# anshmehtamm/ripplemq

Hardware: AMD Instinct MI355X
Metric: committed msgs/sec (node) + HBM GB/s, 100B msgs, 4096 partitions RF=3 (higher is better)
Workload: dtype u8

## Files before the change

### ripplemq_amd/csrc/device_common.hpp

```cpp
#pragma once
#include <hip/hip_runtime.h>
#include <stdint.h>

namespace rmq {

typedef uint32_t u32;
typedef uint64_t u64;
typedef __attribute__((address_space(1))) u64 gu64;
typedef __attribute__((address_space(1))) u32 gu32;

__device__ __forceinline__ void store_sc1(u64* p, u64 v) {
  __hip_atomic_store((gu64*)p, v, __ATOMIC_RELAXED, __HIP_MEMORY_SCOPE_AGENT);
}
__device__ __forceinline__ u64 load_sc1(const u64* p) {
  return __hip_atomic_load((gu64*)p, __ATOMIC_RELAXED, __HIP_MEMORY_SCOPE_AGENT);
}

constexpr u32 kCrcPoly = 0x82F63B78u;
constexpr u32 kRecAlign = 16;

struct CrcConsts {
  u32 table[8][256];
  u32 zshift[2][4][256];
  u32 zshift1k[4][256];
  u32 inv_pad[16];
  u32 sh16[64];
  u32 inv_pad16[16];
  u32 nib[16][32];
};

__host__ __device__ __forceinline__ constexpr u32 record_bytes(u32 len) {
  return 16u + ((len + kRecAlign - 1u) & ~(kRecAlign - 1u));
}

typedef u32 u32x4 __attribute__((ext_vector_type(4)));
typedef u32 u32x2 __attribute__((ext_vector_type(2)));

#ifndef RMQ_RING_NT
#define RMQ_RING_NT 1
#endif
#ifndef RMQ_PAYLOAD_NT
#define RMQ_PAYLOAD_NT 1
#endif
__device__ __forceinline__ uint4 load_payload16(const void* src) {
#if RMQ_PAYLOAD_NT
  const u32x4 x = __builtin_nontemporal_load(reinterpret_cast<const u32x4*>(src));
  return make_uint4(x[0], x[1], x[2], x[3]);
#else
  return *reinterpret_cast<const uint4*>(src);
#endif
}

typedef __attribute__((address_space(1))) const u32x4 gu32x4c;
__device__ __forceinline__ uint4 load_payload16g(u64 addr) {
#if RMQ_PAYLOAD_NT
  const u32x4 x = __builtin_nontemporal_load((gu32x4c*)addr);
#else
  const u32x4 x = *(gu32x4c*)addr;
#endif
  return make_uint4(x[0], x[1], x[2], x[3]);
}

__device__ __forceinline__ void store_log16(uint8_t* dst, uint4 v) {
#if RMQ_RING_NT
  const u32x4 x = {v.x, v.y, v.z, v.w};
  __builtin_nontemporal_store(x, reinterpret_cast<u32x4*>(dst));
#else
  *reinterpret_cast<uint4*>(dst) = v;
#endif
}

__device__ __forceinline__ u32 lane_id() { return __builtin_amdgcn_mbcnt_hi(~0u, __builtin_amdgcn_mbcnt_lo(~0u, 0u)); }


__device__ __forceinline__ u32 gf2_mulmod(u32 a, u32 b) {
  u32 p = 0;
#pragma unroll
  for (int k = 31; k >= 0; --k) {
    p ^= b & (0u - ((a >> k) & 1u));
    b = (b >> 1) ^ (kCrcPoly & (0u - (b & 1u)));
  }
  return p;
}

__device__ __forceinline__ u32 gf2_mulmod_half(u32 a16, u32 b) {
  u32 p = 0;
#pragma unroll
  for (int k = 15; k >= 0; --k) {
    p ^= b & (0u - ((a16 >> k) & 1u));
    b = (b >> 1) ^ (kCrcPoly & (0u - (b & 1u)));
  }
  return p;
}

__device__ __forceinline__ u32 crc_step8(const u32 (*t)[256], u32 c, u32 lo, u32 hi) {
  lo ^= c;
  return t[7][lo & 0xFF] ^ t[6][(lo >> 8) & 0xFF] ^ t[5][(lo >> 16) & 0xFF] ^ t[4][lo >> 24] ^
         t[3][hi & 0xFF] ^ t[2][(hi >> 8) & 0xFF] ^ t[1][(hi >> 16) & 0xFF] ^ t[0][hi >> 24];
}

__device__ __forceinline__ u32 crc_zshift(const u32 (*z)[256], u32 c) {
  return z[0][c & 0xFF] ^ z[1][(c >> 8) & 0xFF] ^ z[2][(c >> 16) & 0xFF] ^ z[3][c >> 24];
}

template <u32 kThreads>
__device__ __forceinline__ void crc_nib_lds(const CrcConsts* crc, u32* scratch) {
  static_assert(sizeof(CrcConsts::nib) == 128 * 16 && kThreads >= 128, "one 16-byte block per thread");
  if (threadIdx.x < 128u)
    reinterpret_cast<uint4*>(scratch)[threadIdx.x] = reinterpret_cast<const uint4*>(&crc->nib[0][0])[threadIdx.x];
  __syncthreads();
}
constexpr u32 kNibBlocks = 128u, kPadBlocks = 4u;
template <u32 kThreads>
__device__ __forceinline__ uint4 crc_nib_load(const CrcConsts* crc) {
  static_assert(sizeof(CrcConsts::nib) == kNibBlocks * 16 && kThreads >= kNibBlocks + 2u * kPadBlocks, "one block per thread");
  static_assert(sizeof(CrcConsts::inv_pad) == kPadBlocks * 16 && sizeof(CrcConsts::inv_pad16) == kPadBlocks * 16, "pad tables");
  const u32 t = threadIdx.x;
  uint4 v = make_uint4(0, 0, 0, 0);
  if (t < kNibBlocks + 2u * kPadBlocks) {
    const uint4* src = t < kNibBlocks ? reinterpret_cast<const uint4*>(&crc->nib[0][0]) + t
                       : t < kNibBlocks + kPadBlocks
                           ? reinterpret_cast<const uint4*>(&crc->inv_pad[0]) + (t - kNibBlocks)
                           : reinterpret_cast<const uint4*>(&crc->inv_pad16[0]) + (t - kNibBlocks - kPadBlocks);
    v = *src;
  }
  return v;
}
__device__ __forceinline__ void crc_nib_put(u32* scratch, u32* pads, uint4 v) {
  const u32 t = threadIdx.x;
  if (t < kNibBlocks)
    reinterpret_cast<uint4*>(scratch)[t] = v;
  else if (t < kNibBlocks + 2u * kPadBlocks)
    reinterpret_cast<uint4*>(pads)[t - kNibBlocks] = v;
}
template <u32 kThreads>
__device__ __forceinline__ void crc_expand_lds(u32* tabs, const u32* scratch) {
  for (u32 b = threadIdx.x; b < 256u; b += kThreads) {
#pragma unroll
    for (u32 q = 0; q < 16u; ++q) tabs[256u * q + b] = scratch[32u * q + (b & 15u)] ^ scratch[32u * q + 16u + (b >> 4)];
  }
}
template <u32 kThreads>
__device__ __forceinline__ void crc_tables_lds(const CrcConsts* crc, u32* tabs, u32* scratch) {
  crc_nib_lds<kThreads>(crc, scratch);
  crc_expand_lds<kThreads>(tabs, scratch);
}

__device__ __forceinline__ u32 crc_piece16(const u32 (*t)[256], uint4 v) {
  return crc_step8(t, crc_step8(t, 0u, v.x, v.y), v.z, v.w);
}

__device__ __forceinline__ u32 pair_swap(u32 v) {
  return (u32)__builtin_amdgcn_update_dpp(0, (int)v, 0xB1, 0xF, 0xF, true);
}


template <int kCtrl, int kRowMask>
__device__ __forceinline__ u32 dpp_mov(u32 v) {
  return (u32)__builtin_amdgcn_update_dpp(0, (int)v, kCtrl, kRowMask, 0xf, true);
}
template <int kCtrl, int kRowMask>
__device__ __forceinline__ u64 dpp_mov(u64 v) {
  return ((u64)dpp_mov<kCtrl, kRowMask>((u32)(v >> 32)) << 32) | dpp_mov<kCtrl, kRowMask>((u32)v);
}

__device__ __forceinline__ u64 bcast_u64(u64 v, u32 l) {
  return ((u64)(u32)__builtin_amdgcn_readlane((int)(v >> 32), (int)l) << 32) |
         (u32)__builtin_amdgcn_readlane((int)(u32)v, (int)l);
}

template <typename T>
__device__ __forceinline__ T wave_incl_scan(T v) {
// ... 84 lines not shown
```

### ripplemq_amd/csrc/engine.cpp

```cpp
#include <chrono>
#include <climits>

#include "engine_internal.hpp"

using namespace rmq;

namespace rmq {

uint32_t host_mulmod(uint32_t a, uint32_t b) {
  uint32_t p = 0;
  for (int k = 31; k >= 0; --k) {
    if ((a >> k) & 1u) p ^= b;
    b = (b >> 1) ^ (kCrcPoly & (0u - (b & 1u)));
  }
  return p;
}

uint32_t host_inverse(uint32_t a) {
  uint32_t col[32];
  for (int k = 0; k < 32; ++k) col[k] = host_mulmod(1u << k, a);
  uint32_t rows[32];
  uint32_t rhs = 0;
  for (int bb = 0; bb < 32; ++bb) {
    rows[bb] = 0;
// ... 19 lines not shown
    ++r;
  }
  uint32_t y = 0;
  for (int q = 0; q < r; ++q)
    if ((rhs >> q) & 1u) y |= 1u << piv[q];
  return y;
}

void build_crc_consts(CrcConsts* c) {
  for (uint32_t b = 0; b < 256; ++b) {
    uint32_t x = b;
    for (int k = 0; k < 8; ++k) x = (x >> 1) ^ (kCrcPoly & (0u - (x & 1u)));
    c->table[0][b] = x;
  }
  for (uint32_t t = 1; t < 8; ++t)
    for (uint32_t b = 0; b < 256; ++b)
      c->table[t][b] = (c->table[t - 1][b] >> 8) ^ c->table[0][c->table[t - 1][b] & 0xFF];
  uint32_t x2n[40];
  x2n[0] = 0x40000000u;
  for (int k = 1; k < 40; ++k) x2n[k] = host_mulmod(x2n[k - 1], x2n[k - 1]);
  for (uint32_t k = 0; k < 2; ++k)
    for (uint32_t i = 0; i < 4; ++i)
      for (uint32_t b = 0; b < 256; ++b) c->zshift[k][i][b] = host_mulmod(b << (8 * i), x2n[7 + k]);
  for (uint32_t i = 0; i < 4; ++i)
    for (uint32_t b = 0; b < 256; ++b) c->zshift1k[i][b] = host_mulmod(b << (8 * i), x2n[13]);
  uint32_t x128e = 0x80000000u;
  for (uint32_t e = 0; e < 64; ++e) {
    c->sh16[e] = x128e;
    x128e = host_mulmod(x128e, x2n[7]);
  }
  uint32_t x8n = 0x80000000u;
  for (uint32_t n = 0; n < 16; ++n) {
    c->inv_pad[n] = n ? host_inverse(x8n) : 0x80000000u;
    c->inv_pad16[n] = host_mulmod(c->inv_pad[n], x2n[4]);
    x8n = host_mulmod(x8n, x2n[3]);
  }
  for (uint32_t q = 0; q < 16; ++q) {
    const uint32_t* t = q < 8 ? c->table[q] : c->zshift[(q - 8) / 4][(q - 8) % 4];
    for (uint32_t n = 0; n < 16; ++n) {
      c->nib[q][n] = t[n];
      c->nib[q][16 + n] = t[n << 4];
    }
  }
}

bool is_pow2(uint64_t v) { return v && !(v & (v - 1)); }

uint32_t ilog2(uint64_t v) {
  uint32_t r = 0;
  while ((1ull << r) < v) ++r;
  return r;
}

int check_err(rmq_engine* e) {
  const hipError_t q = hipStreamQuery(e->main_s);
  return q == hipSuccess || q == hipErrorNotReady ? RMQ_OK : hip_fail(q);
}

template <typename T>
static int spin_then_block(T what, hipError_t (*query)(T), hipError_t (*block)(T)) {
  const auto t0 = std::chrono::steady_clock::now();
  for (;;) {
    const hipError_t q = query(what);
    if (q == hipSuccess) return RMQ_OK;
    if (q != hipErrorNotReady) return hip_fail(q);
    if (std::chrono::steady_clock::now() - t0 > std::chrono::milliseconds(20)) break;
  }
// ... 518 lines not shown
```

### ripplemq_amd/csrc/pipeline.hip

```cpp
#include <hip/hip_ext.h>

#include "device_common.hpp"
#include "kernels.hpp"
#include "partition_ops.hpp"


#ifndef RMQ_PIPE_NS
#define RMQ_PIPE_NS rmq
#endif
namespace RMQ_PIPE_NS {
using namespace rmq;

constexpr u32 kPT = kPipeThreads;
constexpr u32 kPW = kPT / 64;
constexpr u32 kTR = kTileRecs;
constexpr u32 kTI = kTR / kPT;
constexpr u32 kWR = kTR / kPW;
constexpr u32 kIB = kTileIdxBits;
constexpr u32 kFlagShift = 29;
constexpr u32 kRankMask = (1u << kFlagShift) - 1u;
constexpr u32 kFlNoPart = 1u, kFlInvalid = 4u, kFlJunk = 7u;
constexpr u64 kOne40 = 1ull << 40;
constexpr u64 kCnt23 = (1ull << 23) - 1ull;
constexpr u64 kExclNoSpace = 1ull << 63;
constexpr u32 kRejInvalid = 2u;

#define PIPE_STAMP_ROW(row, k)                                                                \
  do {                                                                                        \
    if (A.stamps) {                                                                           \
      const u64 t_ = __builtin_amdgcn_s_memrealtime();                                        \
      if ((threadIdx.x & 63) == 0)                                                            \
        A.stamps[((u64)(row) * kPW + (threadIdx.x >> 6)) * 8 + (k)] = t_;                    \
    }                                                                                         \
  } while (0)
#define PIPE_STAMP(k) PIPE_STAMP_ROW(blockIdx.x, k)

struct Stage1Smem {
  u32 items[2][kTR];
  u32 cnt[kPW][256];
  u32 dbase[256];
  u32 info[kTR];
  u64 wsum[kPW][2];
  u64 wtail[kPW];
  u32 whead[kPW];
  u32 scan[kPW];
};

struct Stage3Smem {
  u32 t8[8][256];
  u32 z[2][4][256];
  uint4 img[kPW][kTaskRecs][8];
  uint4 info[kPW][kTaskRecs];
  u32 pad[2][16];
  union {
    u32 zk[4][256];
    struct {
      u64 xdst[kPW][kTaskRecs][kMaxRemote];
      u32 xn[kPW][kTaskRecs];
    };
  };
};

constexpr size_t kSmemBytes = sizeof(Stage1Smem) > sizeof(Stage3Smem) ? sizeof(Stage1Smem) : sizeof(Stage3Smem);
static_assert(kSmemBytes >= kMaxTiles * sizeof(u64), "stage 2's tile bases fit the dynamic LDS");
static_assert(kPT != 256 || 4 * kSmemBytes <= 160 * 1024, "four 256-thread workgroups per CU fit the 160 KB of LDS");

__device__ __forceinline__ u64 wave_incl_scan_u64(u64 v) { return wave_incl_scan<u64>(v); }

__device__ __forceinline__ u32 record_rs16(u32 L) {
  return (L >> 4) + ((L & 15u) ? 1u : 0u) + 1u;
}

__device__ __forceinline__ u32 batch_of_tile(const PipeGroup& G, u32 t) {
  u32 j = 0;
#pragma unroll
  for (u32 k = 1; k < kMaxGroup; ++k) j += (k < G.nb && t >= G.tile0[k]) ? 1u : 0u;
  return j;
}
__device__ __forceinline__ u32 batch_of_task(const PipeGroup& G, u32 task) {
  u32 j = 0;
#pragma unroll
  for (u32 k = 1; k < kMaxGroup; ++k) j += (k < G.nb && task >= G.task0[k]) ? 1u : 0u;
  return j;
}
__device__ __forceinline__ u32 batch_end_tile(const PipeGroup& G, u32 t) {
  u32 e = G.tiles;
#pragma unroll
  for (int k = (int)kMaxGroup - 1; k >= 1; --k)
    if ((u32)k < G.nb && t < G.tile0[k]) e = G.tile0[k];
  return e;
}

constexpr u32 kBigPieces = 64;
constexpr u32 kBU = 4;

__device__ __forceinline__ u64 readlane64(u64 v, u32 l) {
  return ((u64)(u32)__builtin_amdgcn_readlane((int)(v >> 32), (int)l) << 32) |
         (u32)__builtin_amdgcn_readlane((int)(u32)v, (int)l);
// ... 1343 lines not shown
}

__device__ __forceinline__ void big_close(const PipeArgs& A, const BigRec& R, u32 acc) {
  const u32 lane = threadIdx.x & 63, RF = A.st.RF;
  if (((lane + 64u - R.ph) & 63u) < R.m) {
    const u32 e = (R.m - 1u - lane + R.ph) & 63u;
    if (e) acc = gf2_mulmod(acc, A.crc->sh16[e]);
  }
  acc = wave_xor_all(acc);
  if (lane == 0) {
    const u32 pad = 16u * R.m - R.L;
    const u32 crc = ~(pad ? gf2_mulmod(A.crc->inv_pad[pad], acc) : acc);
    const uint4 h = make_uint4((u32)R.off, (u32)(R.off >> 32), R.L, crc);
    uint8_t* ring = reinterpret_cast<uint8_t*>(R.ring);
    if (R.dead == 0u)
      for (u32 r = 0; r < RF; ++r)
        if ((R.lm >> r) & 1u) store_log16(ring + (R.pos & R.segm) + r * A.st.rstride, h);
#pragma unroll
    for (u32 q = 0; q < kMaxRemote; ++q)
      if (q < R.nx) store_log16(reinterpret_cast<uint8_t*>(R.x[q]), h);
  }
}

template <bool XR>
__device__ __forceinline__ void stage3_big_waves(const PipeArgs& A, Stage3Smem& S, u32 wg) {
  const PipeGroup& G = A.g3;
  const PipeScratch& x = A.s3;
  const DevState& st = A.st;
  const u32 nbig = __builtin_amdgcn_readfirstlane(*reinterpret_cast<volatile const u32*>(x.nbig));
  if (!nbig) return;
  {
    const uint4* src = reinterpret_cast<const uint4*>(&A.crc->table[0][0]);
    uint4* dst = reinterpret_cast<uint4*>(&S.t8[0][0]);
    for (u32 k = threadIdx.x; k < (sizeof(S.t8) + sizeof(S.z)) / 16u; k += kPT) dst[k] = src[k];
    if (!XR) {
      const uint4* zs = reinterpret_cast<const uint4*>(&A.crc->zshift1k[0][0]);
      uint4* zd = reinterpret_cast<uint4*>(&S.zk[0][0]);
      for (u32 k = threadIdx.x; k < sizeof(S.zk) / 16u; k += kPT) zd[k] = zs[k];
    }
  }
  __syncthreads();
  const u32 nw = A.wgb * kPW, lane = threadIdx.x & 63u;
  const u32 e0 = __builtin_amdgcn_readfirstlane(wg * kPW + (threadIdx.x >> 6));
  for (u32 base = e0; base < nbig; base += 64u * nw) {
    const u32 e = base + lane * nw;
    bool ok = e < nbig;
    u64 src = 0, pos = 0, off = 0, ringb = 0, segm = 0;
    u32 L = 0, dead = 0, lm = 0, nx = 0;
    u64 xdst[kMaxRemote] = {};
    if (ok) {
      const u32 gi = x.bigl[e];
      const u32 t = gi / kTR, jb = batch_of_tile(G, t);
      const PipeBatch& b = G.b[jb];
      const u32 i = (t - G.tile0[jb]) * kTR + gi % kTR;
      const uint2 cr = x.crank[gi];
      ok = !(u32)A.s3.binfo[jb * 4] && (cr.x >> kFlagShift) == 0u;
      const u32 p = b.pidx[i];
      L = b.len[i];
      src = reinterpret_cast<u64>(b.payload) + (b.poff ? b.poff[i] : x.tile_base[t] + x.pre[gi]);
      const u64 ex = ok ? x.excl[(u64)p * A.gt + t] : 0ull;
      ok = ok && st.is_leader[p] && !(ex & kExclNoSpace);
      if (ok) {
        const u64 tot = x.totals[p], leo = A.cur.leo[p], used = A.cur.used[p];
        const u32 rk = (u32)((ex >> 40) & kCnt23) + (cr.x & kRankMask);
        const u32 rel16 = (u32)(ex & kLow40) + cr.y;
        off = leo + rk;
        pos = used + 16ull * rel16;
// ... 69 lines not shown

template <bool XR>
__device__ __forceinline__ void stage3_finish(const PipeArgs& A, const Stage3Smem& S, const TaskPos& T, const TaskRec& R,
                              const TaskState& Z, bool cand, uint4& stat_out) {
  const PipeBatch& b = A.g3.b[T.jb];
  const DevState& st = A.st;
  const u32 lane = threadIdx.x & 63, j = lane & 1u;
  const u32 RF = st.RF;
  const u32 i = task_rec(T);
  const bool in = i < b.n;
  const u32 p = R.p, L = R.L;
  const u32 fl = R.cr.x >> kFlagShift;
  const u32 rej = R.rej;
  const bool ns = (Z.lm & kNoSpace) != 0u;
  const bool lead = (Z.lm & kLead) != 0u;
  const u32 lm8 = Z.lm & 0xFFu;
  const bool ok = cand && lead && !ns;
  const u32 m = (L + 15u) >> 4;
  const bool big = ok && m > kBigPieces;
  const bool okp = ok && !big;
  const RingRef rg = ring_ref(Z.rdesc, st.interval_log2, st.icap_mul);
  const u64 segmask = rg.seg - 1ull;
  const u64 rstride = st.rstride;
  const u64 off = Z.off, pos = Z.pos;
  const u32 dead = Z.dead;
  uint8_t* const ring = st.logs + rg.base;
  const u32 lmw = (A.debug & 1u) ? 0u : lm8;
  const u32 sa = (u32)(R.src & 15u);
  u32 acc = 0;
  const u32 nr = okp ? (m + kPR - 1u) / kPR : 0u;
  const bool img = __all(!okp || m <= 7u);
  const u32 w = threadIdx.x >> 6, r32 = lane >> 1;
  Stage3Smem& W = const_cast<Stage3Smem&>(S);
  constexpr bool xr = XR;
  if (xr) {
    if (j == 0) {
      u32 nx = 0;
      if (ok) {
        const u64 rel = 16ull * Z.rel16;
        const u64 rk = Z.rk;
        for (u32 r = 0; r < RF; ++r) {
          if ((lm8 >> r) & 1u) continue;
          const u32 e = A.outidx[(u64)p * RF + r];
          if (e == ~0u) continue;
          const XEntry x = A.xe3[e];
          if (x.data_abs == kNoRound) continue;
          W.xdst[w][r32][nx++] = reinterpret_cast<u64>(A.outbox3 + x.data_abs + rel);
          *reinterpret_cast<u64*>(A.outbox3 + x.tab_abs + 8ull * rk) =
              (u64)x.k | ((u64)(x.data_start16 + (u32)(rel >> 4)) << 32);
        }
      }
      W.xn[w][r32] = nx;
    }
    __builtin_amdgcn_wave_barrier();
  }
  uint4 blk[kBL];
#pragma unroll
  for (u32 q = 0; q < kBL; ++q) blk[q] = Z.blk[q];
  if (Z.nblk) {
    uint4* sg = &W.img[w][0][0];
    static_assert(sizeof(S.img[0]) >= 64u * kSpanPer * 16u, "a wave's image area holds the staged span");
#pragma unroll
    for (u32 u = 0; u < kSpanPer; ++u)
      if (lane + 64u * u < Z.nblk) sg[lane + 64u * u] = Z.blk[u];
    __builtin_amdgcn_wave_barrier();
    const u32 b0 = (u32)(((R.src & ~15ull) - Z.sbase) >> 4) + j;
#pragma unroll
    for (u32 q = 0; q < kBL; ++q) {
      const u32 k = b0 + 2u * q;
      blk[q] = k < Z.nblk ? sg[k] : make_uint4(0, 0, 0, 0);
    }
    __builtin_amdgcn_wave_barrier();
  }
  for (u32 c = 0; __any(c < nr); ++c) {
    if (c) round_blocks(A, R, c, c < nr, blk);
#pragma unroll
    for (u32 q = 0; q < 4; ++q) {
      const uint4 pb = pair_swap4(j ? blk[q] : blk[q + 1]);
      const u32 jp = kPR * c + j + 2u * q;
      if (c < nr && jp < m) {
        const u32 nb = L - 16u * jp < 16u ? L - 16u * jp : 16u;
        const uint4 v = extract_piece(blk[q], pb, sa, nb);
        acc = crc_zshift(S.z[1], acc) ^ piece_crc(A, S, v, jp);
        if (img) {
          const_cast<Stage3Smem&>(S).img[w][r32][jp + 1] = v;
        } else {
          uint8_t* dst = ring + ((pos + 16ull + 16ull * jp) & segmask);
          if (jp + 1u >= dead)
            for (u32 r = 0; r < RF; ++r)
              if ((lmw >> r) & 1u) store_log16(dst + r * rstride, v);
          if (xr)
            for (u32 q = 0; q < S.xn[w][r32]; ++q)
              store_log16(reinterpret_cast<uint8_t*>(S.xdst[w][r32][q]) + 16ull + 16ull * jp, v);
        }
      }
    }
  }
  if (okp && m > j && ((m - 1u - j) & 1u)) acc = crc_zshift(S.z[0], acc);
  acc ^= pair_swap(acc);

  u32 part = 0;
  if (okp && L) {
    const u32 pad = 16u * m - L;
    part = pad ? gf2_mulmod_half(j ? acc & 0xFFFFu : acc >> 16, S.pad[j][pad]) : (j ? 0u : acc);
  }
  part ^= pair_swap(part);
  uint4 h = make_uint4(0, 0, 0, 0);
  if (okp && j == 1) h = make_uint4((u32)off, (u32)(off >> 32), L, L ? ~part : 0u);
  if (img) {
    if (j == 1) W.img[w][r32][0] = h;
    if (j == 0)
      W.info[w][r32] = make_uint4((u32)pos, (u32)(pos >> 32), (u32)(rg.base >> 8),
                                  okp ? lm8 | (m << 8) | (1u << 12) | (dead << 13) | ((u32)(Z.rdesc & 63ull) << 24) : 0u);
    __builtin_amdgcn_wave_barrier();
#pragma unroll
    for (u32 s4 = 0; s4 < kTaskRecs * 8u / 64u; ++s4) {
      const u32 idx = lane + 64u * s4, rr = idx >> 3, k = idx & 7u;
      const uint4 inf = W.info[w][rr];
      const u32 mr = (inf.w >> 8) & 0xFu;
      if (((inf.w >> 12) & 1u) && k <= mr) {
        const uint4 v = W.img[w][rr][k];
        if (k >= ((inf.w >> 13) & 0x1Fu)) {
          const u64 rpos = ((u64)inf.y << 32) | inf.x;
          const u64 rmask = (1ull << (inf.w >> 24)) - 1ull;
          uint8_t* dst = st.logs + ((u64)inf.z << 8) + ((rpos + 16ull * k) & rmask);
          const u32 lmr = (A.debug & 1u) ? 0u : (inf.w & 0xFFu);
          for (u32 r = 0; r < RF; ++r)
            if ((lmr >> r) & 1u) store_log16(dst + r * rstride, v);
        }
        if (xr)
          for (u32 q = 0; q < W.xn[w][rr]; ++q) store_log16(reinterpret_cast<uint8_t*>(W.xdst[w][rr][q]) + 16ull * k, v);
      }
    }
    __builtin_amdgcn_wave_barrier();
  } else if (okp && j == 1) {
    uint8_t* dst = ring + (pos & segmask);
    if (dead == 0u)
      for (u32 r = 0; r < RF; ++r)
        if ((lm8 >> r) & 1u) store_log16(dst + r * rstride, h);
    if (xr)
      for (u32 q = 0; q < S.xn[w][r32]; ++q) store_log16(reinterpret_cast<uint8_t*>(S.xdst[w][r32][q]), h);
  }
  if (in && j == 0) b.out_offsets[i] = ok ? off : ~0ull;
  const u32 ilog = st.interval_log2;
  const u64 end = pos + 16ull * (1ull + m);
  if (ok && j == 1) {
    for (u64 mm = (pos >> ilog) + 1; (mm << ilog) <= end; ++mm) {
      u64* e = st.index + (rg.ibase + mm % rg.icap) * 2;
      e[0] = off + 1;
      e[1] = end;
    }
  }
  {
    const bool h0 = j == 0;
    const u32 n_in = (u32)__popcll(__ballot(h0 && in));
    const u32 n_app = (u32)__popcll(__ballot(h0 && ok));
    const u32 n_nl = (u32)__popcll(__ballot(h0 && cand && !lead));
    const u32 n_np = rej ? 0u : (u32)__popcll(__ballot(h0 && in && fl == kFlNoPart));
    const u32 n_inv = (rej & kRejInvalid) ? n_in : 0u;
    const u32 n_ns = (u32)__popcll(__ballot(h0 && cand && lead && ns));
    stat_out = make_uint4(n_app, n_nl, n_np, n_ns | (n_inv << 16));
  }
}

__device__ __forceinline__ void partition_threads(const PipeArgs& A, u32 p) {
  const DevState& st = A.st;
  const u32 RF = st.RF;
  const bool a3 = A.g3.nb != 0, a4 = A.g4.nb != 0;
  const bool lead = st.is_leader[p];
  const u64 tot3 = a3 ? A.s3.totals[p] : 0ull;
  const u64 leo0 = A.cur.leo[p], used0 = A.cur.used[p];
  const u32 lm = st.local_mask[p];
  u64 row[kMaxRF];
#pragma unroll
// ... 77 lines not shown
    const u64 m = (c.pos >> ilog) + j;
    const u64 w0 = j ? m << ilog : c.pos, w1 = min(end, (m + 1ull) << ilog);
    u64 roff = c.first, rpos = c.pos;
    if (j) {
      const u64* ie = st.index + (rg.ibase + m % rg.icap) * 2;
      roff = ie[0];
      rpos = ie[1];
    }
    for (u64 sub = w0 & ~1023ull; sub < w1; sub += 1024) {
      const u64 q = sub + 16ull * lane;
      uint4 v = make_uint4(0, 0, 0, 0);
      const bool mine = q >= w0 && q < w1;
      if (mine) {
        v = *reinterpret_cast<const uint4*>(ring + (q & mask));
        store_log16(A.outbox3 + c.data_abs + (q - c.pos), v);
      }
      while (rpos < min(sub + 1024ull, w1)) {
        const u32 L = (u32)__shfl((int)v.z, (int)((rpos - sub) >> 4), 64);
        if (lane == 0)
          *reinterpret_cast<u64*>(A.outbox3 + c.tab_abs + 8ull * (roff - c.first)) =
              (u64)c.k | ((u64)(c.data_start16 + (u32)((rpos - c.pos) >> 4)) << 32);
        rpos += 16ull + ((L + 15ull) & ~15ull);
        ++roff;
      }
    }
  }
}

#ifndef RMQ_S3_LOADERS
#define RMQ_S3_LOADERS 3
#endif
constexpr u32 kS3Loaders = RMQ_S3_LOADERS;
constexpr u32 kS3Storers = kPW > kS3Loaders ? kPW - kS3Loaders : 1u;
constexpr u32 kS3Bufs = 4;
struct Stage3RSmem {
  u32 t8[8][256];
  u32 z[2][4][256];
  uint4 img[kS3Bufs][kTaskRecs][8];
  uint4 info[kS3Bufs][kTaskRecs][2];
  uint4 stat[kS3Bufs];
  u32 seq[kS3Bufs];
};
static_assert(sizeof(Stage3RSmem) <= kSmemBytes, "the role-split stage 3 fits the launch's LDS");
constexpr u32 kRfImg = 8u;
constexpr u32 kRfSt = 1u << 12;
constexpr u32 kRfDead = 13u;
constexpr u32 kRfOk = 1u << 18;
constexpr u32 kRfIn = 1u << 19;

__device__ __forceinline__ u32 lds_seq(const u32* s) {
  return __builtin_amdgcn_readfirstlane(__hip_atomic_load(s, __ATOMIC_RELAXED, __HIP_MEMORY_SCOPE_WORKGROUP));
}
__device__ __forceinline__ void lds_wait_seq(const u32* s, u32 v) {
  for (u32 k = 0; lds_seq(s) < v && k < (1u << 24); ++k) __builtin_amdgcn_s_sleep(1);
  asm volatile("" ::: "memory");
}
__device__ __forceinline__ void lds_post_seq(u32* s, u32 v) {
  asm volatile("s_waitcnt lgkmcnt(0)" ::: "memory");
  if ((threadIdx.x & 63) == 0) __hip_atomic_store(s, v, __ATOMIC_RELAXED, __HIP_MEMORY_SCOPE_WORKGROUP);
}

__device__ __forceinline__ void stage3_build(const PipeArgs& A, Stage3RSmem& S, const TaskPos& T, const TaskRec& R,
                                             const TaskState& Z, bool cand, u32 bi) {
  const PipeBatch& b = A.g3.b[T.jb];
  const DevState& st = A.st;
  const u32 lane = threadIdx.x & 63, j = lane & 1u, r32 = lane >> 1;
  const u32 RF = st.RF;
  const u32 i = task_rec(T);
  const bool in = i < b.n;
  const u32 L = R.L;
  const u32 fl = R.cr.x >> kFlagShift;
  const u32 rej = R.rej;
  const bool ns = (Z.lm & kNoSpace) != 0u;
  const bool lead = (Z.lm & kLead) != 0u;
  const u32 lm8 = Z.lm & 0xFFu;
  const bool ok = cand && lead && !ns;
  const u32 m = (L + 15u) >> 4;
  const bool big = ok && m > kBigPieces;
  const bool okp = ok && !big;
  const RingRef rg = ring_ref(Z.rdesc, st.interval_log2, st.icap_mul);
  const u64 segmask = rg.seg - 1ull;
  const u64 pos = Z.pos;
  uint8_t* const ring = st.logs + rg.base;
  const u32 lmw = (A.debug & 1u) ? 0u : lm8;
  const u32 sa = (u32)(R.src & 15u);
  const u32 nr = okp ? (m + kPR - 1u) / kPR : 0u;
  const bool img = __all(!okp || m <= 7u);
  u32 acc = 0;
  uint4 blk[kBL];
#pragma unroll
  for (u32 q = 0; q < kBL; ++q) blk[q] = Z.blk[q];
  for (u32 c = 0; __any(c < nr); ++c) {
    if (c) round_blocks(A, R, c, c < nr, blk);
#pragma unroll
    for (u32 q = 0; q < 4; ++q) {
      const uint4 pb = pair_swap4(j ? blk[q] : blk[q + 1]);
      const u32 jp = kPR * c + j + 2u * q;
      if (c < nr && jp < m) {
        const u32 nb = L - 16u * jp < 16u ? L - 16u * jp : 16u;
        uint4 v = extract_piece(blk[q], pb, sa, nb);
        uint4 vc = v;
        if (jp == 0) vc.x ^= 0xFFFFFFFFu;
        acc = crc_zshift(S.z[1], acc) ^ ((A.debug & 2u) ? vc.x : crc_piece16(S.t8, vc));
        if (img) {
          S.img[bi][r32][jp + 1] = v;
        } else {
          uint8_t* dst = ring + ((pos + 16ull + 16ull * jp) & segmask);
          if (jp + 1u >= Z.dead)
            for (u32 r = 0; r < RF; ++r)
              if ((lmw >> r) & 1u) store_log16(dst + r * st.rstride, v);
        }
      }
    }
  }
  if (okp && m > j && ((m - 1u - j) & 1u)) acc = crc_zshift(S.z[0], acc);
  acc ^= pair_swap(acc);
  u32 part = 0;
  if (okp && L) {
    const u32 pad = 16u * m - L;
    part = pad ? gf2_mulmod_half(j ? acc & 0xFFFFu : acc >> 16, j ? A.crc->inv_pad16[pad] : A.crc->inv_pad[pad])
               : (j ? 0u : acc);
  }
  part ^= pair_swap(part);
  if (j == 1) {
    S.img[bi][r32][0] = okp ? make_uint4((u32)Z.off, (u32)(Z.off >> 32), L, L ? ~part : 0u) : make_uint4(0, 0, 0, 0);
  } else {
    const u32 f = (okp ? (lmw | ((img ? m : 0u) << kRfImg) | kRfSt) : 0u) | (min(Z.dead, 31u) << kRfDead) |
                  (ok ? kRfOk : 0u) | (in ? kRfIn : 0u);
    S.info[bi][r32][0] = make_uint4((u32)pos, (u32)(pos >> 32), (u32)Z.off, (u32)(Z.off >> 32));
    S.info[bi][r32][1] = make_uint4((u32)Z.rdesc, (u32)(Z.rdesc >> 32), f, m);
  }
  const bool h0 = j == 0;
  const u32 n_in = (u32)__popcll(__ballot(h0 && in));
  const u32 n_app = (u32)__popcll(__ballot(h0 && ok));
  const u32 n_nl = (u32)__popcll(__ballot(h0 && cand && !lead));
  const u32 n_np = rej ? 0u : (u32)__popcll(__ballot(h0 && in && fl == kFlNoPart));
  const u32 n_inv = (rej & kRejInvalid) ? n_in : 0u;
  const u32 n_ns = (u32)__popcll(__ballot(h0 && cand && lead && ns));
  if (lane == 0) S.stat[bi] = make_uint4(n_app, n_nl, n_np, n_ns | (n_inv << 16));
}

__device__ __forceinline__ void stage3_store(const PipeArgs& A, Stage3RSmem& S, u32 task, u32 bi, u32 ti) {
  const PipeGroup& G = A.g3;
  const DevState& st = A.st;
  const u32 lane = threadIdx.x & 63;
  const TaskPos T = task_pos(G, task);
  const PipeBatch& b = G.b[T.jb];
  constexpr u32 kS4 = kTaskRecs * 8u / 64u;
  uint4 v[kS4], i0[kS4], i1[kS4];
#pragma unroll
  for (u32 s4 = 0; s4 < kS4; ++s4) {
    const u32 idx = lane + 64u * s4, rr = idx >> 3, k = idx & 7u;
    v[s4] = S.img[bi][rr][k];
    i0[s4] = S.info[bi][rr][0];
// ... 7 lines not shown
#pragma unroll
  for (u32 s4 = 0; s4 < kS4; ++s4) {
    const u32 k = (lane + 64u * s4) & 7u;
    const u32 f = i1[s4].z;
    if ((f & kRfSt) && k <= ((f >> kRfImg) & 0xFu) && k >= ((f >> kRfDead) & 31u)) {
      const u64 rpos = ((u64)i0[s4].y << 32) | i0[s4].x;
      const RingRef rg = ring_ref(((u64)i1[s4].y << 32) | i1[s4].x, st.interval_log2, st.icap_mul);
      uint8_t* dst = st.logs + rg.base + ((rpos + 16ull * k) & (rg.seg - 1ull));
      for (u32 r = 0; r < st.RF; ++r)
        if ((f >> r) & 1u) store_log16(dst + r * rstride, v[s4]);
    }
  }
  if (lane < kTaskRecs) {
    const u32 f = r1.z;
    const u64 off = ((u64)r0.w << 32) | r0.z;
    if (f & kRfIn) b.out_offsets[T.i0 + lane] = (f & kRfOk) ? off : ~0ull;
    if (f & kRfOk) {
      const u32 ilog = st.interval_log2;
      const u64 pos = ((u64)r0.y << 32) | r0.x;
      const u64 end = pos + 16ull * (1ull + r1.w);
      const RingRef rg = ring_ref(((u64)r1.y << 32) | r1.x, ilog, st.icap_mul);
      for (u64 mm = (pos >> ilog) + 1; (mm << ilog) <= end; ++mm) {
        u64* e = st.index + (rg.ibase + mm % rg.icap) * 2;
        e[0] = off + 1;
        e[1] = end;
      }
    }
  }
  if (lane == 0) G.stats[T.jb][task - G.task0[T.jb]] = so;
}

__device__ __forceinline__ void roles_tables(const PipeArgs& A, Stage3RSmem& S) {
  static_assert(offsetof(CrcConsts, zshift) == sizeof(A.crc->table), "table and zshift adjacent");
  constexpr u32 kN = (sizeof(S.t8) + sizeof(S.z)) / 16u, kT = kS3Loaders * 64u, kPer = (kN + kT - 1u) / kT;
  const uint4* src = reinterpret_cast<const uint4*>(&A.crc->table[0][0]);
  uint4* dst = reinterpret_cast<uint4*>(&S.t8[0][0]);
  uint4 v[kPer];
#pragma unroll
  for (u32 q = 0; q < kPer; ++q) v[q] = src[min(threadIdx.x + q * kT, kN - 1u)];
#pragma unroll
  for (u32 q = 0; q < kPer; ++q)
    if (threadIdx.x + q * kT < kN) dst[threadIdx.x + q * kT] = v[q];
}

__device__ __forceinline__ void stage3_roles(const PipeArgs& A, Stage3RSmem& S, u32 slot) {
  const PipeGroup& G = A.g3;
  const u32 tasks = G.task0[G.nb];
  const u32 t0 = (u32)((u64)slot * tasks / A.wg3), n = (u32)((u64)(slot + 1u) * tasks / A.wg3) - t0;
  const u32 w = __builtin_amdgcn_readfirstlane(threadIdx.x >> 6);
  PIPE_STAMP(0);
  if (w < kS3Loaders && w < n) {
    u32 i = w;
    TaskPos T = task_pos(G, t0 + i);
    TaskRec R = stage3_r1(A, T);
    if (!(A.debug & 8u)) roles_tables(A, S);
    bool cand = stage3_cand(A, T, R);
    TaskState Z = stage3_r2(A, T, R, cand);
    if (threadIdx.x < kS3Bufs) S.seq[threadIdx.x] = 0u;
    __syncthreads();
    PIPE_STAMP(1);
    u64 waited = 0, tw = 0;
    for (;;) {
      const u32 in_ = i + kS3Loaders;
      const bool more = in_ < n;
      TaskPos Tn = T;
      TaskRec Rn = R;
      if (more) {
        Tn = task_pos(G, t0 + in_);
        Rn = stage3_r1(A, Tn);
      }
      const u32 bi = i % kS3Bufs;
      if (A.stamps) tw = __builtin_amdgcn_s_memrealtime();
// ... 120 lines not shown
    PIPE_STAMP(0);
    if (wg == 0 && A.g4.nb) {
      if (threadIdx.x < 4) A.s4.nbig[threadIdx.x] = 0u;
      if (threadIdx.x < kMaxGroup * 2) A.s4.bacc[threadIdx.x] = 0ull;
    }
    for (u32 p = wg * kPT + threadIdx.x; p < A.st.P; p += A.wgp * kPT) partition_threads(A, p);
    if (A.stamps) asm volatile("s_waitcnt vmcnt(0)" ::: "memory");
    PIPE_STAMP(6);
    return;
  }
  Stage3Smem& S = *reinterpret_cast<Stage3Smem*>(smem_raw);
  const PipeGroup& G = A.g3;
  sgpr_fetch(G.nb, G.task0[0], G.task0[1], G.task0[2], G.task0[3], G.task0[4], G.task0[5], G.task0[6], G.task0[7],
             G.task0[8], A.s3_xcd, A.s3_lead, A.s3_roles, A.s3_pair);
  static_assert(kMaxGroup == 8, "the task table's entries above");
  u32 tasks = G.task0[0];
#pragma unroll
  for (u32 k = 1; k <= kMaxGroup; ++k) tasks = G.nb == k ? G.task0[k] : tasks;
  const u32 lane = threadIdx.x & 63;
  const u32 slot = A.s3_xcd ? xcd_rank(A.s3_lead ? 0u : A.wg1 + A.wg2 + A.wgp, A.wg3, blockIdx.x) : wg;
  if (!XR && A.s3_roles) {
    stage3_roles(A, *reinterpret_cast<Stage3RSmem*>(smem_raw), slot);
    return;
  }
  u32 task = __builtin_amdgcn_readfirstlane(slot * kPW + (threadIdx.x >> 6));
  PIPE_STAMP(0);
  if (!XR && A.s3_pair) {
    const u32 tb = task + A.wg3 * kPW;
    const bool ha = task < tasks, hb = tb < tasks;
    const TaskPos Ta = task_pos(G, ha ? task : 0u), Tb = task_pos(G, hb ? tb : 0u);
    const uint4 nv = crc_nib_load<kPT>(A.crc);
    const TaskRec Ra = stage3_r1(A, Ta), Rb = stage3_r1(A, Tb);
    if (!(A.debug & 8u)) {
      crc_nib_put(reinterpret_cast<u32*>(&S.img[0][0][0]), &S.pad[0][0], nv);
      __syncthreads();
      crc_expand_lds<kPT>(&S.t8[0][0], reinterpret_cast<const u32*>(&S.img[0][0][0]));
    }
    const bool ca = ha && stage3_cand(A, Ta, Ra), cb = hb && stage3_cand(A, Tb, Rb);
    const TaskState Za = stage3_r2(A, Ta, Ra, ca);
    const TaskState Zb = stage3_r2(A, Tb, Rb, cb);
    __syncthreads();
    uint4 so;
    if (ha) {
      stage3_finish<XR>(A, S, Ta, Ra, Za, ca, so);
      if (lane == 0) G.stats[Ta.jb][task - G.task0[Ta.jb]] = so;
    }
    if (hb) {
      stage3_finish<XR>(A, S, Tb, Rb, Zb, cb, so);
      if (lane == 0) G.stats[Tb.jb][tb - G.task0[Tb.jb]] = so;
    }
    return;
  }
  TaskPos T = task_pos(G, task < tasks ? task : 0u);
  {
    const PipeBatch& b = G.b[T.jb];
    sgpr_fetch(b.pidx, b.len, b.poff, b.payload, b.n, G.tile0[T.jb], A.s3.crank, A.s3.pre, A.s3.tile_base, A.s3.binfo);
  }
  const uint4 nv = crc_nib_load<kPT>(A.crc);
  TaskRec R = stage3_r1(A, T);
  static_assert(offsetof(Stage3Smem, z) == sizeof(S.t8), "t8 and z adjacent in LDS");
  if (!(A.debug & 8u)) crc_nib_put(reinterpret_cast<u32*>(&S.img[0][0][0]), &S.pad[0][0], nv);
  bool cand = task < tasks && stage3_cand(A, T, R);
  RecRaw W0;
  TaskState Z = stage3_r2(A, T, R, cand, A.s3_stage != 0u, &W0);
  __syncthreads();
  if (!(A.debug & 8u)) crc_expand_lds<kPT>(&S.t8[0][0], reinterpret_cast<const u32*>(&S.img[0][0][0]));
  stage3_place(Z, W0, R, cand);
  __syncthreads();
  PIPE_STAMP(1);
  while (task < tasks) {
    uint4 so;
    PIPE_STAMP(2);
    stage3_finish<XR>(A, S, T, R, Z, cand, so);
    if (lane == 0) G.stats[T.jb][task - G.task0[T.jb]] = so;
    PIPE_STAMP(3);
    task += A.wg3 * kPW;
    if (task < tasks) {
      T = task_pos(G, task);
      R = stage3_r1(A, T);
      cand = stage3_cand(A, T, R);
      Z = stage3_r2(A, T, R, cand, A.s3_stage != 0u);
    }
  }
  if (A.stamps) asm volatile("s_waitcnt vmcnt(0)" ::: "memory");
  PIPE_STAMP(6);
  if (A.steal && A.g1.nb && !(A.debug & 16u)) {
    __syncthreads();
    stage1_tiles(A, smem_raw, 0, true);
  }
}

#ifdef RMQ_PIPE_XR_TU
void launch_pipeline_xr(const PipeArgs& a, hipStream_t s, hipEvent_t start) {
  const u32 grid = a.wg1 + a.wg2 + a.wgp + a.wg3 + a.wgb + a.wgc;
  hipExtLaunchKernelGGL(pipeline_kernel<true>, dim3(grid), dim3(kPT), kSmemBytes, s, start, nullptr, 0, a);
}
#else
uint32_t pipeline_wgs_per_cu(uint32_t threads) { return RMQ_PIPE_WAVES_PER_SIMD * 4u / (threads / 64u); }

// ... 15 lines not shown
```

Baseline: 6.618 billion.

## Fold odd-parity CRC shift into pad constants and shrink stage-3 LDS

```diff
diff --git a/ripplemq_amd/csrc/device_common.hpp b/ripplemq_amd/csrc/device_common.hpp
--- a/ripplemq_amd/csrc/device_common.hpp
+++ b/ripplemq_amd/csrc/device_common.hpp
@@ -25,7 +25,7 @@
   u32 zshift1k[4][256];
   u32 inv_pad[16];
   u32 sh16[64];
-  u32 inv_pad16[16];
+  u32 pair_pad[2][2][16];
   u32 nib[16][32];
 };
 
@@ -92,6 +92,17 @@
   }
   return p;
 }
+__device__ __forceinline__ u32 gf2_mulmod_half2(u32 a16, u32 b, u32 c16, u32 d) {
+  u32 p = 0, q = 0;
+#pragma unroll
+  for (int k = 15; k >= 0; --k) {
+    p ^= b & (0u - ((a16 >> k) & 1u));
+    q ^= d & (0u - ((c16 >> k) & 1u));
+    b = (b >> 1) ^ (kCrcPoly & (0u - (b & 1u)));
+    d = (d >> 1) ^ (kCrcPoly & (0u - (d & 1u)));
+  }
+  return p ^ q;
+}
 
 __device__ __forceinline__ u32 crc_step8(const u32 (*t)[256], u32 c, u32 lo, u32 hi) {
   lo ^= c;
@@ -110,18 +121,16 @@
     reinterpret_cast<uint4*>(scratch)[threadIdx.x] = reinterpret_cast<const uint4*>(&crc->nib[0][0])[threadIdx.x];
   __syncthreads();
 }
-constexpr u32 kNibBlocks = 128u, kPadBlocks = 4u;
+constexpr u32 kNibTabs = 12u, kNibBlocks = kNibTabs * 8u, kPadBlocks = 16u;
 template <u32 kThreads>
 __device__ __forceinline__ uint4 crc_nib_load(const CrcConsts* crc) {
-  static_assert(sizeof(CrcConsts::nib) == kNibBlocks * 16 && kThreads >= kNibBlocks + 2u * kPadBlocks, "one block per thread");
-  static_assert(sizeof(CrcConsts::inv_pad) == kPadBlocks * 16 && sizeof(CrcConsts::inv_pad16) == kPadBlocks * 16, "pad tables");
+  static_assert(sizeof(CrcConsts::nib) == 16 * 8 * 16 && kThreads >= kNibBlocks + kPadBlocks, "one block per thread");
+  static_assert(sizeof(CrcConsts::pair_pad) == kPadBlocks * 16, "pad tables");
   const u32 t = threadIdx.x;
   uint4 v = make_uint4(0, 0, 0, 0);
-  if (t < kNibBlocks + 2u * kPadBlocks) {
-    const uint4* src = t < kNibBlocks ? reinterpret_cast<const uint4*>(&crc->nib[0][0]) + t
-                       : t < kNibBlocks + kPadBlocks
-                           ? reinterpret_cast<const uint4*>(&crc->inv_pad[0]) + (t - kNibBlocks)
-                           : reinterpret_cast<const uint4*>(&crc->inv_pad16[0]) + (t - kNibBlocks - kPadBlocks);
+  if (t < kNibBlocks + kPadBlocks) {
+    const uint4* src = t < kNibBlocks ? reinterpret_cast<const uint4*>(&crc->nib[0][0]) + (t < 64u ? t : t + 32u)
+                                      : reinterpret_cast<const uint4*>(&crc->pair_pad[0][0][0]) + (t - kNibBlocks);
     v = *src;
   }
   return v;
@@ -130,14 +139,14 @@
   const u32 t = threadIdx.x;
   if (t < kNibBlocks)
     reinterpret_cast<uint4*>(scratch)[t] = v;
-  else if (t < kNibBlocks + 2u * kPadBlocks)
+  else if (t < kNibBlocks + kPadBlocks)
     reinterpret_cast<uint4*>(pads)[t - kNibBlocks] = v;
 }
-template <u32 kThreads>
+template <u32 kThreads, u32 kTabs = 16u>
 __device__ __forceinline__ void crc_expand_lds(u32* tabs, const u32* scratch) {
   for (u32 b = threadIdx.x; b < 256u; b += kThreads) {
 #pragma unroll
-    for (u32 q = 0; q < 16u; ++q) tabs[256u * q + b] = scratch[32u * q + (b & 15u)] ^ scratch[32u * q + 16u + (b >> 4)];
+    for (u32 q = 0; q < kTabs; ++q) tabs[256u * q + b] = scratch[32u * q + (b & 15u)] ^ scratch[32u * q + 16u + (b >> 4)];
   }
 }
 template <u32 kThreads>
diff --git a/ripplemq_amd/csrc/engine.cpp b/ripplemq_amd/csrc/engine.cpp
--- a/ripplemq_amd/csrc/engine.cpp
+++ b/ripplemq_amd/csrc/engine.cpp
@@ -75,7 +75,11 @@
   uint32_t x8n = 0x80000000u;
   for (uint32_t n = 0; n < 16; ++n) {
     c->inv_pad[n] = n ? host_inverse(x8n) : 0x80000000u;
-    c->inv_pad16[n] = host_mulmod(c->inv_pad[n], x2n[4]);
+    for (uint32_t r = 0; r < 2; ++r) {
+      const uint32_t v = r ? host_mulmod(c->inv_pad[n], x2n[7]) : c->inv_pad[n];
+      c->pair_pad[0][r][n] = v;
+      c->pair_pad[1][r][n] = host_mulmod(v, x2n[4]);
+    }
     x8n = host_mulmod(x8n, x2n[3]);
   }
   for (uint32_t q = 0; q < 16; ++q) {
diff --git a/ripplemq_amd/csrc/pipeline.hip b/ripplemq_amd/csrc/pipeline.hip
--- a/ripplemq_amd/csrc/pipeline.hip
+++ b/ripplemq_amd/csrc/pipeline.hip
@@ -48,22 +48,33 @@
 
 struct Stage3Smem {
   u32 t8[8][256];
-  u32 z[2][4][256];
-  uint4 img[kPW][kTaskRecs][8];
+  u32 z[4][256];
+  union {
+    uint4 img[kPW][kTaskRecs][8];
+    u32 zk[4][256];
+  };
   uint4 info[kPW][kTaskRecs];
-  u32 pad[2][16];
-  union {
-    u32 zk[4][256];
-    struct {
-      u64 xdst[kPW][kTaskRecs][kMaxRemote];
-      u32 xn[kPW][kTaskRecs];
-    };
-  };
+  u32 pad[2][2][16];
 };
-
-constexpr size_t kSmemBytes = sizeof(Stage1Smem) > sizeof(Stage3Smem) ? sizeof(Stage1Smem) : sizeof(Stage3Smem);
+static_assert(sizeof(Stage3Smem::zk) <= sizeof(Stage3Smem::img), "the 1 KB shift table fits the image area it overlays");
+
+struct Stage3XSmem {
+  u64 xdst[kPW][kTaskRecs][kMaxRemote];
+  u32 xn[kPW][kTaskRecs];
+};
+static_assert(sizeof(Stage3Smem) % 16 == 0, "Stage3XSmem follows Stage3Smem aligned");
+__device__ __forceinline__ Stage3XSmem& stage3_x(const Stage3Smem& S) {
+  return *reinterpret_cast<Stage3XSmem*>(const_cast<Stage3Smem*>(&S) + 1);
+}
+
+#ifdef RMQ_PIPE_XR_TU
+constexpr size_t kStage3Bytes = sizeof(Stage3Smem) + sizeof(Stage3XSmem);
+#else
+constexpr size_t kStage3Bytes = sizeof(Stage3Smem);
+#endif
+constexpr size_t kSmemBytes = sizeof(Stage1Smem) > kStage3Bytes ? sizeof(Stage1Smem) : kStage3Bytes;
 static_assert(kSmemBytes >= kMaxTiles * sizeof(u64), "stage 2's tile bases fit the dynamic LDS");
-static_assert(kPT != 256 || 4 * kSmemBytes <= 160 * 1024, "four 256-thread workgroups per CU fit the 160 KB of LDS");
+static_assert(kPT != 256 || 5 * kSmemBytes <= 160 * 1024, "five 256-thread workgroups per CU fit the 160 KB of LDS");
 
 __device__ __forceinline__ u64 wave_incl_scan_u64(u64 v) { return wave_incl_scan<u64>(v); }
 
@@ -1473,7 +1484,7 @@
   {
     const uint4* src = reinterpret_cast<const uint4*>(&A.crc->table[0][0]);
     uint4* dst = reinterpret_cast<uint4*>(&S.t8[0][0]);
-    for (u32 k = threadIdx.x; k < (sizeof(S.t8) + sizeof(S.z)) / 16u; k += kPT) dst[k] = src[k];
+    for (u32 k = threadIdx.x; k < sizeof(S.t8) / 16u; k += kPT) dst[k] = src[k];
     if (!XR) {
       const uint4* zs = reinterpret_cast<const uint4*>(&A.crc->zshift1k[0][0]);
       uint4* zd = reinterpret_cast<uint4*>(&S.zk[0][0]);
@@ -1609,6 +1620,7 @@
   const bool img = __all(!okp || m <= 7u);
   const u32 w = threadIdx.x >> 6, r32 = lane >> 1;
   Stage3Smem& W = const_cast<Stage3Smem&>(S);
+  Stage3XSmem& X = stage3_x(S);
   constexpr bool xr = XR;
   if (xr) {
     if (j == 0) {
@@ -1622,12 +1634,12 @@
           if (e == ~0u) continue;
           const XEntry x = A.xe3[e];
           if (x.data_abs == kNoRound) continue;
-          W.xdst[w][r32][nx++] = reinterpret_cast<u64>(A.outbox3 + x.data_abs + rel);
+          X.xdst[w][r32][nx++] = reinterpret_cast<u64>(A.outbox3 + x.data_abs + rel);
           *reinterpret_cast<u64*>(A.outbox3 + x.tab_abs + 8ull * rk) =
               (u64)x.k | ((u64)(x.data_start16 + (u32)(rel >> 4)) << 32);
         }
       }
-      W.xn[w][r32] = nx;
+      X.xn[w][r32] = nx;
     }
     __builtin_amdgcn_wave_barrier();
   }
@@ -1658,7 +1670,7 @@
       if (c < nr && jp < m) {
         const u32 nb = L - 16u * jp < 16u ? L - 16u * jp : 16u;
         const uint4 v = extract_piece(blk[q], pb, sa, nb);
-        acc = crc_zshift(S.z[1], acc) ^ piece_crc(A, S, v, jp);
+        acc = crc_zshift(S.z, acc) ^ piece_crc(A, S, v, jp);
         if (img) {
           const_cast<Stage3Smem&>(S).img[w][r32][jp + 1] = v;
         } else {
@@ -1667,19 +1679,18 @@
             for (u32 r = 0; r < RF; ++r)
               if ((lmw >> r) & 1u) store_log16(dst + r * rstride, v);
           if (xr)
-            for (u32 q = 0; q < S.xn[w][r32]; ++q)
-              store_log16(reinterpret_cast<uint8_t*>(S.xdst[w][r32][q]) + 16ull + 16ull * jp, v);
+            for (u32 q = 0; q < X.xn[w][r32]; ++q)
+              store_log16(reinterpret_cast<uint8_t*>(X.xdst[w][r32][q]) + 16ull + 16ull * jp, v);
         }
       }
     }
   }
-  if (okp && m > j && ((m - 1u - j) & 1u)) acc = crc_zshift(S.z[0], acc);
-  acc ^= pair_swap(acc);
-
+  const u32 pacc = pair_swap(acc);
   u32 part = 0;
   if (okp && L) {
-    const u32 pad = 16u * m - L;
-    part = pad ? gf2_mulmod_half(j ? acc & 0xFFFFu : acc >> 16, S.pad[j][pad]) : (j ? 0u : acc);
+    const u32 pad = 16u * m - L, row = (m - 1u - j) & 1u;
+    part = gf2_mulmod_half2(j ? acc & 0xFFFFu : acc >> 16, S.pad[j][row][pad],
+                            j ? pacc & 0xFFFFu : pacc >> 16, S.pad[j][row ^ 1u][pad]);
   }
   part ^= pair_swap(part);
   uint4 h = make_uint4(0, 0, 0, 0);
@@ -1706,7 +1717,7 @@
             if ((lmr >> r) & 1u) store_log16(dst + r * rstride, v);
         }
         if (xr)
-          for (u32 q = 0; q < W.xn[w][rr]; ++q) store_log16(reinterpret_cast<uint8_t*>(W.xdst[w][rr][q]) + 16ull * k, v);
+          for (u32 q = 0; q < X.xn[w][rr]; ++q) store_log16(reinterpret_cast<uint8_t*>(X.xdst[w][rr][q]) + 16ull * k, v);
       }
     }
     __builtin_amdgcn_wave_barrier();
@@ -1716,7 +1727,7 @@
       for (u32 r = 0; r < RF; ++r)
         if ((lm8 >> r) & 1u) store_log16(dst + r * rstride, h);
     if (xr)
-      for (u32 q = 0; q < S.xn[w][r32]; ++q) store_log16(reinterpret_cast<uint8_t*>(S.xdst[w][r32][q]), h);
+      for (u32 q = 0; q < X.xn[w][r32]; ++q) store_log16(reinterpret_cast<uint8_t*>(X.xdst[w][r32][q]), h);
   }
   if (in && j == 0) b.out_offsets[i] = ok ? off : ~0ull;
   const u32 ilog = st.interval_log2;
@@ -1860,10 +1871,10 @@
 #endif
 constexpr u32 kS3Loaders = RMQ_S3_LOADERS;
 constexpr u32 kS3Storers = kPW > kS3Loaders ? kPW - kS3Loaders : 1u;
-constexpr u32 kS3Bufs = 4;
+constexpr u32 kS3Bufs = 3;
 struct Stage3RSmem {
   u32 t8[8][256];
-  u32 z[2][4][256];
+  u32 z[4][256];
   uint4 img[kS3Bufs][kTaskRecs][8];
   uint4 info[kS3Bufs][kTaskRecs][2];
   uint4 stat[kS3Bufs];
@@ -1929,7 +1940,7 @@
         uint4 v = extract_piece(blk[q], pb, sa, nb);
         uint4 vc = v;
         if (jp == 0) vc.x ^= 0xFFFFFFFFu;
-        acc = crc_zshift(S.z[1], acc) ^ ((A.debug & 2u) ? vc.x : crc_piece16(S.t8, vc));
+        acc = crc_zshift(S.z, acc) ^ ((A.debug & 2u) ? vc.x : crc_piece16(S.t8, vc));
         if (img) {
           S.img[bi][r32][jp + 1] = v;
         } else {
@@ -1941,13 +1952,12 @@
       }
     }
   }
-  if (okp && m > j && ((m - 1u - j) & 1u)) acc = crc_zshift(S.z[0], acc);
-  acc ^= pair_swap(acc);
+  const u32 pacc = pair_swap(acc);
   u32 part = 0;
   if (okp && L) {
-    const u32 pad = 16u * m - L;
-    part = pad ? gf2_mulmod_half(j ? acc & 0xFFFFu : acc >> 16, j ? A.crc->inv_pad16[pad] : A.crc->inv_pad[pad])
-               : (j ? 0u : acc);
+    const u32 pad = 16u * m - L, row = (m - 1u - j) & 1u;
+    part = gf2_mulmod_half2(j ? acc & 0xFFFFu : acc >> 16, A.crc->pair_pad[j][row][pad],
+                            j ? pacc & 0xFFFFu : pacc >> 16, A.crc->pair_pad[j][row ^ 1u][pad]);
   }
   part ^= pair_swap(part);
   if (j == 1) {
@@ -2021,12 +2031,17 @@
 
 __device__ __forceinline__ void roles_tables(const PipeArgs& A, Stage3RSmem& S) {
   static_assert(offsetof(CrcConsts, zshift) == sizeof(A.crc->table), "table and zshift adjacent");
+  static_assert(offsetof(Stage3RSmem, z) == sizeof(S.t8), "t8 and z adjacent in LDS");
   constexpr u32 kN = (sizeof(S.t8) + sizeof(S.z)) / 16u, kT = kS3Loaders * 64u, kPer = (kN + kT - 1u) / kT;
+  constexpr u32 kT8 = sizeof(S.t8) / 16u, kSkip = sizeof(A.crc->zshift[0]) / 16u;
   const uint4* src = reinterpret_cast<const uint4*>(&A.crc->table[0][0]);
   uint4* dst = reinterpret_cast<uint4*>(&S.t8[0][0]);
   uint4 v[kPer];
 #pragma unroll
-  for (u32 q = 0; q < kPer; ++q) v[q] = src[min(threadIdx.x + q * kT, kN - 1u)];
+  for (u32 q = 0; q < kPer; ++q) {
+    const u32 k = min(threadIdx.x + q * kT, kN - 1u);
+    v[q] = src[k < kT8 ? k : k + kSkip];
+  }
 #pragma unroll
   for (u32 q = 0; q < kPer; ++q)
     if (threadIdx.x + q * kT < kN) dst[threadIdx.x + q * kT] = v[q];
@@ -2213,9 +2228,9 @@
     const uint4 nv = crc_nib_load<kPT>(A.crc);
     const TaskRec Ra = stage3_r1(A, Ta), Rb = stage3_r1(A, Tb);
     if (!(A.debug & 8u)) {
-      crc_nib_put(reinterpret_cast<u32*>(&S.img[0][0][0]), &S.pad[0][0], nv);
+      crc_nib_put(reinterpret_cast<u32*>(&S.img[0][0][0]), &S.pad[0][0][0], nv);
       __syncthreads();
-      crc_expand_lds<kPT>(&S.t8[0][0], reinterpret_cast<const u32*>(&S.img[0][0][0]));
+      crc_expand_lds<kPT, kNibTabs>(&S.t8[0][0], reinterpret_cast<const u32*>(&S.img[0][0][0]));
     }
     const bool ca = ha && stage3_cand(A, Ta, Ra), cb = hb && stage3_cand(A, Tb, Rb);
     const TaskState Za = stage3_r2(A, Ta, Ra, ca);
@@ -2239,13 +2254,14 @@
   }
   const uint4 nv = crc_nib_load<kPT>(A.crc);
   TaskRec R = stage3_r1(A, T);
-  static_assert(offsetof(Stage3Smem, z) == sizeof(S.t8), "t8 and z adjacent in LDS");
-  if (!(A.debug & 8u)) crc_nib_put(reinterpret_cast<u32*>(&S.img[0][0][0]), &S.pad[0][0], nv);
+  static_assert(offsetof(Stage3Smem, z) == sizeof(S.t8) && sizeof(S.t8) + sizeof(S.z) == kNibTabs * 1024u,
+                "t8 and z adjacent in LDS: the twelve tables crc_expand_lds builds");
+  if (!(A.debug & 8u)) crc_nib_put(reinterpret_cast<u32*>(&S.img[0][0][0]), &S.pad[0][0][0], nv);
   bool cand = task < tasks && stage3_cand(A, T, R);
   RecRaw W0;
   TaskState Z = stage3_r2(A, T, R, cand, A.s3_stage != 0u, &W0);
   __syncthreads();
-  if (!(A.debug & 8u)) crc_expand_lds<kPT>(&S.t8[0][0], reinterpret_cast<const u32*>(&S.img[0][0][0]));
+  if (!(A.debug & 8u)) crc_expand_lds<kPT, kNibTabs>(&S.t8[0][0], reinterpret_cast<const u32*>(&S.img[0][0][0]));
   stage3_place(Z, W0, R, cand);
   __syncthreads();
   PIPE_STAMP(1);
```

After: 6.421 billion. 0.97x the previous value.
